# christopherkarani/Wax

Measured on AMD Instinct MI355X. Metric: queries/sec, 10M x 384-dim f32 cosine top-10 brute-force scan (single query per step), higher is better.
Workload: dtype f32; 1 GPU; 10M x 384 f32 unit-Gaussian corpus in HBM, cosine top-10, 1 query/step; rows=10000000, dims=384, top_k=10, rows_per_gpu=10000000, pipeline_depth=4, merge=device, exchange=none, rccl_ranks=0, parallelism=row-shard x1, checksum=4db467d0ff1310ca

## Files before the change

wax_amd/csrc/mirror_pass.h:

```cpp
#pragma once
#include <cstddef>
#include <type_traits>

#include "kernels.h"
#include "row_math.h"
#include "topk.h"

namespace wax {

typedef float f32x2 __attribute__((ext_vector_type(2)));

using MirrorDims = DimList<384, 768>;

constexpr int MIRROR_CAP = 128;
constexpr int MIRROR_PASS_LDS = SCAN_WAVES * MIRROR_CAP + SCAN_WAVES + MIRROR_KP;

template <class ROWS, int DIMS>
struct MirrorShape {
    static constexpr int D8 = DIMS / 8;
    static constexpr int GROUP = D8 / 3, LOADS = 3;
    static constexpr int RPW = WAVE / GROUP, RPC = RPW * ROWS::UNROLL;
    static_assert(D8 % GROUP == 0 && D8 / GROUP == LOADS, "three load vectors per lane and row");
};

template <class ARGSQ>
struct LoneQuery {
    const MirrorScanArgs& a;
    static __device__ __forceinline__ const f32x4* kernarg_floats() {
        return reinterpret_cast<const f32x4*>((const char*)__builtin_amdgcn_kernarg_segment_ptr() + offsetof(ARGSQ, q));
    }
    __device__ __forceinline__ const f32x4* floats(int) const { return kernarg_floats(); }
    __device__ __forceinline__ float norm(int) const { return a.q_norm; }
    __device__ __forceinline__ int64_t* partials(int) const { return a.partials; }
};
struct MemberQueries {
    const MirrorMember* m;
    __device__ __forceinline__ const f32x4* floats(int i) const { return reinterpret_cast<const f32x4*>(m[i].query); }
    __device__ __forceinline__ float norm(int i) const { return m[i].q_norm; }
    __device__ __forceinline__ int64_t* partials(int i) const { return m[i].partials; }
    __device__ __forceinline__ const uint32_t* bitmap(int i) const { return m[i].bitmap; }
};
__device__ __forceinline__ MirrorScanArgs member_args(MirrorScanArgs a, const MirrorMember& m) {
    a.partials = m.partials;
    a.hits = m.hits;
    a.certified = m.certified;
    a.q_norm = m.q_norm;
    a.k = m.k;
    a.kpad = m.kpad;
    return a;
}

struct NoClock {
    __device__ __forceinline__ void begin() {}
    __device__ __forceinline__ void loop_begin() {}
    __device__ __forceinline__ void prune_in() {}
    __device__ __forceinline__ void prune_out() {}
    __device__ __forceinline__ void loop_end() {}
    __device__ __forceinline__ void done() {}
};
template <bool SORTED_, class CLOCK_ = NoClock>
struct PassFrame {
    static constexpr bool SORTED = SORTED_;
    using Clock = CLOCK_;
};
using FramePlain = PassFrame<false>;
using FrameShipped = PassFrame<true>;

template <int NQ, class FRAME = FrameShipped>
struct PassLists {
    static_assert(NQ >= 1 && NQ <= MIRROR_MAX_NQ, "queries per pass");
    WaveTopK<MIRROR_CAP> tk[NQ];
    unsigned full;
    int64_t* lds;
    int wave;
    typename FRAME::Clock clk;

    __device__ __forceinline__ void init(int64_t* lds_, int wave_) {
        lds = lds_;
        wave = wave_;
#pragma unroll
        for (int i = 0; i < NQ; ++i) tk[i].init(lds + i * MIRROR_PASS_LDS + wave * MIRROR_CAP, MIRROR_KP);
        full = 0u;
    }

    __device__ __forceinline__ void pruned(int i, int cnt, int64_t tau) {
        tk[i].cnt = __builtin_amdgcn_readfirstlane(cnt);
        const uint32_t lo = (uint32_t)__builtin_amdgcn_readfirstlane((int)(uint32_t)tau);
        const uint32_t hi = (uint32_t)__builtin_amdgcn_readfirstlane((int)(tau >> 32));
        tk[i].tau = (int64_t)(((uint64_t)hi << 32) | lo);
    }
    __device__ __forceinline__ void prune(int i) {
        if constexpr (FRAME::SORTED) {
            if ((full >> i) & 1u) {
                if (tk[i].cnt == MIRROR_KP) return;
                const PruneOut r = wave_prune_sorted<MIRROR_CAP>((lds_i64*)tk[i].buf, tk[i].cnt);
                pruned(i, r.cnt, r.tau);
                return;
            }
        }
        const PruneOut r = wave_prune<MIRROR_CAP, true>((lds_i64*)tk[i].buf, tk[i].cnt, tk[i].k);
        pruned(i, r.cnt, r.tau);
        if constexpr (FRAME::SORTED) full |= (tk[i].cnt == MIRROR_KP ? 1u : 0u) << i;
    }

    __device__ __forceinline__ void room(int rows) {
        bool shortof = false;
#pragma unroll
        for (int i = 0; i < NQ; ++i) shortof = shortof || tk[i].cnt > MIRROR_CAP - rows;
        if (shortof) {
            clk.prune_in();
#pragma unroll
            for (int i = 0; i < NQ; ++i)
                if (tk[i].cnt > MIRROR_CAP - rows) prune(i);
            clk.prune_out();
        }
    }

    __device__ __forceinline__ void offer(int i, int64_t key, bool valid) { tk[i].push(key, valid); }

    template <class QUERIES>
    __device__ __forceinline__ void finish(const QUERIES& qs) {
        clk.loop_end();
        const int lane = lane_id();
#pragma unroll
        for (int i = 0; i < NQ; ++i) {
            prune(i);
            int* counts = reinterpret_cast<int*>(lds + i * MIRROR_PASS_LDS + SCAN_WAVES * MIRROR_CAP);
            if (lane == 0) counts[wave] = tk[i].cnt;
        }
        __syncthreads();
#pragma unroll
        for (int i = 0; i < NQ; ++i) {
            int64_t* base = lds + i * MIRROR_PASS_LDS;
            block_rank_merge<SCAN_WAVES>(base, MIRROR_CAP, reinterpret_cast<int*>(base + SCAN_WAVES * MIRROR_CAP), MIRROR_KP,
                                         base + SCAN_WAVES * MIRROR_CAP + SCAN_WAVES);
        }
        __syncthreads();
#pragma unroll
        for (int i = 0; i < NQ; ++i) {
            const int64_t* fin = lds + i * MIRROR_PASS_LDS + SCAN_WAVES * MIRROR_CAP + SCAN_WAVES;
            int64_t* mine = qs.partials(i) + (size_t)blockIdx.x * MIRROR_KP;
            for (int t = (int)threadIdx.x; t < MIRROR_KP; t += SCAN_THREADS) mine[t] = fin[t];
        }
        clk.done();
    }
};

template <class ROWS, int DIMS, int METRIC, int NQ, bool MASKED, class QUERIES>
__device__ __forceinline__ void mirror_pass(const typename ROWS::Vec* __restrict__ rows, const typename ROWS::Side* __restrict__ sides,
                                            const MirrorScanArgs& a, const QUERIES& qs, const uint32_t* __restrict__ bitmap, int64_t* lds) {
    using S = MirrorShape<ROWS, DIMS>;
    constexpr int D8 = S::D8, GROUP = S::GROUP, LOADS = S::LOADS, RPW = S::RPW, RPC = S::RPC, UNROLL = ROWS::UNROLL;
    static_assert(NQ >= 1 && NQ <= MIRROR_MAX_NQ, "queries per pass");
    static_assert(!MASKED || ((RPC & (RPC - 1)) == 0 && RPC <= 32), "a chunk's bits must sit inside one bitmap word");

    const int lane = lane_id();
    const int wave = (int)(threadIdx.x >> 6);
    const int sub = lane / GROUP;
    const int gl = lane % GROUP;
    const bool owner = (gl == GROUP - 1);
    const uint32_t n = a.n_rows;

    f32x2 q[NQ][LOADS][4];
    float start[NQ], qn[NQ], inv_qn[NQ];
    PassLists<NQ> lists;
    lists.init(lds, wave);
#pragma unroll
    for (int i = 0; i < NQ; ++i) {
        const f32x4* q4 = qs.floats(i);
#pragma unroll
        for (int j = 0; j < LOADS; ++j) {
            const f32x4 lo = q4[2 * (gl + j * GROUP)], hi = q4[2 * (gl + j * GROUP) + 1];
            q[i][j][0] = lo.xy; q[i][j][1] = lo.zw; q[i][j][2] = hi.xy; q[i][j][3] = hi.zw;
        }
        start[i] = ROWS::start(q[i]);
        qn[i] = qs.norm(i);
        inv_qn[i] = qn[i] > COS_NORM_FLOOR ? 1.0f / qn[i] : 0.0f;
    }

    const uint32_t nchunks = (n + RPC - 1) / RPC;
    const uint32_t gwave = blockIdx.x * SCAN_WAVES + wave;
    const uint32_t nwaves = gridDim.x * SCAN_WAVES;

    uint32_t word = 0u, bits = 0u;
    if constexpr (MASKED) word = gwave < nchunks ? bitmap[(gwave * RPC) >> 5] : 0u;
    for (uint32_t chunk = gwave; chunk < nchunks; chunk += nwaves) {
        if constexpr (MASKED) {
            const uint32_t r0 = chunk * RPC;
            bits = (uint32_t)__builtin_amdgcn_readfirstlane((int)((word >> (r0 & 31u)) & (uint32_t)((1ull << RPC) - 1ull)));
            const uint32_t next = chunk + nwaves;
            if (next < nchunks) word = bitmap[(next * RPC) >> 5];
            if (bits == 0u) continue;
        }
        const uint32_t rbase = chunk * RPC + sub;
        lists.room(RPC);
        typename ROWS::Vec v[UNROLL][LOADS];
        typename ROWS::Side side[UNROLL];
#pragma unroll
        for (int u = 0; u < UNROLL; ++u) {
            const uint32_t r = rbase + u * RPW;
            const uint32_t rc = r < n ? r : n - 1;
            const typename ROWS::Vec* p = rows + (size_t)rc * D8 + gl;
#pragma unroll
            for (int j = 0; j < LOADS; ++j) v[u][j] = __builtin_nontemporal_load(p + j * GROUP);
            side[u] = ROWS::side(sides, rc);
        }
#pragma unroll
        for (int u = 0; u < UNROLL; ++u) {
            const uint32_t r = rbase + u * RPW;
            bool offer = owner && (r < n);
            if constexpr (MASKED) offer = offer && ((bits >> (uint32_t)(sub + u * RPW)) & 1u) != 0u;
#pragma unroll
            for (int i = 0; i < NQ; ++i) {
                f32x2 acc[4] = {{start[i], 0.f}, {0.f, 0.f}, {0.f, 0.f}, {0.f, 0.f}};
#pragma unroll
                for (int j = 0; j < LOADS; ++j) {
                    acc[0] = __builtin_elementwise_fma(q[i][j][0], ROWS::part(v[u][j], 0), acc[0]);
                    acc[1] = __builtin_elementwise_fma(q[i][j][1], ROWS::part(v[u][j], 1), acc[1]);
                    acc[2] = __builtin_elementwise_fma(q[i][j][2], ROWS::part(v[u][j], 2), acc[2]);
                    acc[3] = __builtin_elementwise_fma(q[i][j][3], ROWS::part(v[u][j], 3), acc[3]);
                }
                const f32x2 s2 = (acc[0] + acc[1]) + (acc[2] + acc[3]);
                const float s = group_sum<GROUP>(s2.x + s2.y);
                const float d = ROWS::template key<METRIC>(s, side[u], inv_qn[i], qn[i]);
                lists.offer(i, make_key(d + 0.0f, a.row_base + r), offer);
            }
        }
    }

    lists.finish(qs);
}

inline int mirror_pass_grid(uint32_t n_rows, int rows_per_chunk, int grid_cap) {
    if (grid_cap <= 0) grid_cap = 512;
    if (grid_cap > SCAN_KWAY_MERGE_GRID) grid_cap = SCAN_KWAY_MERGE_GRID;
    const uint64_t rpc = (uint64_t)rows_per_chunk;
    const uint64_t nchunks = ((uint64_t)n_rows + rpc - 1) / rpc;
    const uint64_t max_waves = (uint64_t)grid_cap * SCAN_WAVES;
    uint64_t waves = nchunks;
    if (nchunks > max_waves) {
        const uint64_t iters = (nchunks + max_waves - 1) / max_waves;
        waves = (nchunks + iters - 1) / iters;
    }
    uint64_t blocks = (waves + SCAN_WAVES - 1) / SCAN_WAVES;
    if (blocks < 1) blocks = 1;
    if (blocks > (uint64_t)grid_cap) blocks = grid_cap;
    return (int)blocks;
}

inline bool mirror_launch_ok(const MirrorScanArgs& a, int metric, int max_k, const MirrorMember* m = nullptr, int nq = 1) {
    if (!mirror_scan_supported(a.dims, metric) || a.n_rows == 0) return false;
    if (m == nullptr) return a.k >= 1 && a.k <= max_k && a.kpad >= a.k;
    if (nq < 2 || nq > MIRROR_MAX_NQ) return false;
    for (int i = 0; i < nq; ++i)
        if (m[i].k < 1 || m[i].k > max_k || m[i].kpad < m[i].k || m[i].query == nullptr) return false;
    return true;
}

template <class ROWS, typename F>
inline hipError_t with_mirror_pass(uint32_t n_rows, uint32_t dims, int metric, int grid_cap, F&& launch) {
    return with_scan_shape(MirrorDims{}, dims, [&](auto s) {
        return with_metric_in<M_COS, M_DOT>(metric, [&](auto m) {
            return launch(s, m, mirror_pass_grid(n_rows, MirrorShape<ROWS, decltype(s)::DIMS>::RPC, grid_cap));
        }, hipErrorInvalidValue);
    }, hipErrorInvalidValue);
}

template <typename F>
inline hipError_t with_group_size(int nq, F&& f) {
    switch (nq) {
        case 2: return f(std::integral_constant<int, 2>{});
        case 3: return f(std::integral_constant<int, 3>{});
        case 4: return f(std::integral_constant<int, 4>{});
        default: return hipErrorInvalidValue;
    }
}

template <typename K, typename ARGS>
inline hipError_t launch_finish(K finish, int nq, hipStream_t st, const ARGS& args) {
    hipError_t err = hipGetLastError();
    if (err != hipSuccess) return err;
    hipLaunchKernelGGL(finish, dim3(nq), dim3(SCAN_THREADS), 0, st, args);
    return hipGetLastError();
}

}
```

Before: 5579 queries/s.

## Share a block-wide pruning bound across waves to reject candidates earlier

Each wave publishes, through LDS atomics, the key at a fixed rank in its pruned top list. The block bound is taken as the max over the per-wave values and kept with atomic min. Before offering, every wave reads this shared bound and drops keys that cannot reach the block top-K, so fewer pushes and prunes happen. In exchange it adds LDS atomics, a noinline publish call, a per-room bound read and an extra __syncthreads at init, all enabled by default through FrameShipped.

Result: slower. 3736 queries/s (-33.0%).

```diff
diff --git a/wax_amd/csrc/mirror_pass.h b/wax_amd/csrc/mirror_pass.h
--- a/wax_amd/csrc/mirror_pass.h
+++ b/wax_amd/csrc/mirror_pass.h
@@ -13,7 +13,9 @@
 using MirrorDims = DimList<384, 768>;
 
 constexpr int MIRROR_CAP = 128;
-constexpr int MIRROR_PASS_LDS = SCAN_WAVES * MIRROR_CAP + SCAN_WAVES + MIRROR_KP;
+constexpr int MIRROR_PASS_Q16 = SCAN_WAVES * MIRROR_CAP + SCAN_WAVES + MIRROR_KP;
+constexpr int MIRROR_PASS_LDS = MIRROR_PASS_Q16 + SCAN_WAVES + 1;
+constexpr int MIRROR_BOUND_RANK = MIRROR_KP / SCAN_WAVES;
 
 template <class ROWS, int DIMS>
 struct MirrorShape {
@@ -55,22 +57,38 @@
     __device__ __forceinline__ void loop_begin() {}
     __device__ __forceinline__ void prune_in() {}
     __device__ __forceinline__ void prune_out() {}
+    __device__ __forceinline__ void list_pruned() {}
+    __device__ __forceinline__ void pushed(int) {}
     __device__ __forceinline__ void loop_end() {}
     __device__ __forceinline__ void done() {}
 };
-template <bool SORTED_, class CLOCK_ = NoClock>
+template <bool SORTED_, bool BOUND_, class CLOCK_ = NoClock>
 struct PassFrame {
-    static constexpr bool SORTED = SORTED_;
+    static constexpr bool SORTED = SORTED_, BOUND = BOUND_;
     using Clock = CLOCK_;
 };
-using FramePlain = PassFrame<false>;
-using FrameShipped = PassFrame<true>;
+using FramePlain = PassFrame<false, false>;
+using FrameSorted = PassFrame<true, false>;
+using FrameShipped = PassFrame<true, true>;
+
+__device__ __attribute__((noinline)) inline void pass_publish(const lds_i64* list, lds_i64* q16, int wave) {
+    if (lane_id() != 0) return;
+    __hip_atomic_fetch_min(q16 + wave, list[MIRROR_BOUND_RANK - 1], __ATOMIC_RELAXED, __HIP_MEMORY_SCOPE_WORKGROUP);
+    int64_t most = __hip_atomic_load(q16, __ATOMIC_RELAXED, __HIP_MEMORY_SCOPE_WORKGROUP);
+#pragma unroll
+    for (int w = 1; w < SCAN_WAVES; ++w) {
+        const int64_t o = __hip_atomic_load(q16 + w, __ATOMIC_RELAXED, __HIP_MEMORY_SCOPE_WORKGROUP);
+        most = o > most ? o : most;
+    }
+    __hip_atomic_fetch_min(q16 + SCAN_WAVES, most, __ATOMIC_RELAXED, __HIP_MEMORY_SCOPE_WORKGROUP);
+}
 
 template <int NQ, class FRAME = FrameShipped>
 struct PassLists {
     static_assert(NQ >= 1 && NQ <= MIRROR_MAX_NQ, "queries per pass");
     WaveTopK<MIRROR_CAP> tk[NQ];
     unsigned full;
+    int64_t bound[NQ];
     int64_t* lds;
     int wave;
     typename FRAME::Clock clk;
@@ -81,6 +99,23 @@
 #pragma unroll
         for (int i = 0; i < NQ; ++i) tk[i].init(lds + i * MIRROR_PASS_LDS + wave * MIRROR_CAP, MIRROR_KP);
         full = 0u;
+        if constexpr (FRAME::BOUND) {
+#pragma unroll
+            for (int i = 0; i < NQ; ++i) {
+                bound[i] = KEY_PAD;
+                int64_t* q16 = lds + i * MIRROR_PASS_LDS + MIRROR_PASS_Q16;
+                if (lane_id() == 0) {
+                    q16[wave] = KEY_PAD;
+                    if (wave == 0) q16[SCAN_WAVES] = KEY_PAD;
+                }
+            }
+            __syncthreads();
+        }
+    }
+
+    __device__ __forceinline__ void publish(int i) {
+        if (tk[i].cnt < MIRROR_BOUND_RANK) return;
+        pass_publish((const lds_i64*)tk[i].buf, (lds_i64*)(lds + i * MIRROR_PASS_LDS + MIRROR_PASS_Q16), wave);
     }
 
     __device__ __forceinline__ void pruned(int i, int cnt, int64_t tau) {
@@ -111,12 +146,34 @@
             clk.prune_in();
 #pragma unroll
             for (int i = 0; i < NQ; ++i)
-                if (tk[i].cnt > MIRROR_CAP - rows) prune(i);
+                if (tk[i].cnt > MIRROR_CAP - rows) {
+                    prune(i);
+                    if constexpr (FRAME::BOUND) publish(i);
+                    clk.list_pruned();
+                }
             clk.prune_out();
         }
-    }
-
-    __device__ __forceinline__ void offer(int i, int64_t key, bool valid) { tk[i].push(key, valid); }
+        if constexpr (FRAME::BOUND) {
+            int64_t word[NQ];
+#pragma unroll
+            for (int i = 0; i < NQ; ++i)
+                word[i] = __hip_atomic_load((const lds_i64*)(lds + i * MIRROR_PASS_LDS + MIRROR_PASS_Q16 + SCAN_WAVES), __ATOMIC_RELAXED,
+                                            __HIP_MEMORY_SCOPE_WORKGROUP);
+#pragma unroll
+            for (int i = 0; i < NQ; ++i) {
+                const uint32_t lo = (uint32_t)__builtin_amdgcn_readfirstlane((int)(uint32_t)word[i]);
+                const uint32_t hi = (uint32_t)__builtin_amdgcn_readfirstlane((int)(word[i] >> 32));
+                bound[i] = (int64_t)(((uint64_t)hi << 32) | lo);
+            }
+        }
+    }
+
+    __device__ __forceinline__ void offer(int i, int64_t key, bool valid) {
+        if constexpr (FRAME::BOUND) valid = valid && key < bound[i];
+        const int before = tk[i].cnt;
+        tk[i].push(key, valid);
+        clk.pushed(tk[i].cnt - before);
+    }
 
     template <class QUERIES>
     __device__ __forceinline__ void finish(const QUERIES& qs) {
```
